# TencentARC/SEED-Story

Hardware: AMD Instinct MI355X
Metric: story-steps/sec (text + 1024x1024 image) (higher is better)
Workload: dtype bf16

## Files before the change

### seed-story_amd/csrc/ss_gemm_common.h

```cpp
#pragma once
#include <type_traits>
#include <utility>

#include "ss_common.h"

namespace ss {

typedef __attribute__((ext_vector_type(4))) uint32_t u32x4_t;
typedef __attribute__((ext_vector_type(8))) uint32_t u32x8_t;
template <int NV> struct Frag { uint4 v[NV]; };
template <typename T> struct OutT { using type = T; };
template <> struct OutT<fp8_t> { using type = bf16_t; };
template <typename T> struct Mma;
template <> struct Mma<bf16_t> {
    static constexpr int kK = 32;
    static constexpr int kEB = 2;
    static constexpr int kNV = 1;
    static __device__ __forceinline__ f32x4_t run(const uint4& a, const uint4& b, f32x4_t c) {
        return __builtin_amdgcn_mfma_f32_16x16x32_bf16(__builtin_bit_cast(bf16x8_t, a),
                                                       __builtin_bit_cast(bf16x8_t, b), c, 0, 0, 0);
    }
    static __device__ __forceinline__ void run_inplace(const uint4& a, const uint4& b, f32x4_t& c) {
        asm volatile("v_mfma_f32_16x16x32_bf16 %0, %1, %2, %0"
                     : "+v"(c)
// ... 49 lines not shown
    const float erf_abs = fmaf(-poly * t, e, 1.0f);
    return 0.5f * v + 0.5f * fabsf(v) * erf_abs;
}
template <typename T> __device__ __forceinline__ float gelu_for(float v) {
    if constexpr (Tr<T>::kVec == 8) return gelu_erf16(v);
    else return gelu_erf(v);
}

constexpr int SS_EPI_INTERNAL_GENERIC = 1 << 30;

struct GemmArgs {
    const void* A = nullptr; const void* W = nullptr; void* C = nullptr; const void* bias = nullptr; const void* residual = nullptr;
    int M = 0, N = 0, K = 0;
    int64_t lda = 0, ldw = 0, ldc = 0, ldr = 0;
    int epi = 0;
    const void* rowvec = nullptr; int rows_per_batch = 1; int64_t rowvec_ld = 0;
    int conv_H = 0, conv_W = 0, conv_Cin = 0, conv_stride = 0, conv_up = 0, conv_Ho = 0, conv_Wo = 0;
    int swz = 0;
    const float* scale_a = nullptr; const float* scale_w = nullptr;
    const float* shift_a = nullptr;
    double* rowstat_out = nullptr;
    float* rowpart = nullptr; int rowpart_ld = 0;
    const float* ln_part = nullptr; int ln_nstrip = 0; float ln_inv_width = 0.f, ln_eps = 0.f;
    int ksplit = 1;
};
static_assert(sizeof(GemmArgs) == 224, "GemmArgs is a kernel argument: its layout does not change");

static inline GemmArgs gemm_args(const void* A, const void* W, void* C, int64_t M, int64_t N, int64_t K, int64_t lda, int64_t ldw,
                          int64_t ldc, int epi, const void* bias = nullptr, const void* residual = nullptr, int64_t ldr = 0) {
    GemmArgs g;
    g.A = A; g.W = W; g.C = C; g.bias = bias; g.residual = residual;
    g.M = (int)M; g.N = (int)N; g.K = (int)K; g.lda = lda; g.ldw = ldw; g.ldc = ldc; g.ldr = ldr; g.epi = epi;
    return g;
}

__device__ __forceinline__ void xcd_tile_id(int swz, int MT, int NT, int id, int& mt, int& nt) {
    if (!swz) { mt = id / NT; nt = id - mt * NT; return; }
    const int total = MT * NT;
    const int xcd = id & 7, j = id >> 3;
    const int base = total >> 3, rem = total & 7;
    const int L = xcd * base + (xcd < rem ? xcd : rem) + j;
    const int GM = swz;
    const int per_group = GM * NT;
    const int gidx = L / per_group, r = L - gidx * per_group;
    const int m0 = gidx * GM;
    const int gm = (MT - m0) < GM ? (MT - m0) : GM;
    nt = r / gm;
    mt = m0 + r - nt * gm;
}
__device__ __forceinline__ void xcd_tile(int swz, int MT, int NT, int& mt, int& nt) {
    xcd_tile_id(swz, MT, NT, blockIdx.y * gridDim.x + blockIdx.x, mt, nt);
}


typedef __attribute__((address_space(3))) void lds_void_t;

__device__ __forceinline__ void dma16(const void* gsrc, uint32_t lds_base) {
    uint32_t keep;
    asm volatile(
        "s_mov_b32 %0, m0\n\t"
        "s_mov_b32 m0, %2\n\t"
        "s_nop 0\n\t"
        "global_load_lds_dwordx4 %1, off\n\t"
        "s_mov_b32 m0, %0"
        : "=&s"(keep)
        : "v"(gsrc), "s"(lds_base)
        : "memory");
}
__device__ __forceinline__ uint32_t m0_save() {
    uint32_t keep;
    asm volatile("s_mov_b32 %0, m0" : "=s"(keep)::"memory");
    return keep;
}
__device__ __forceinline__ void m0_restore(uint32_t keep) { asm volatile("s_mov_b32 m0, %0" ::"s"(keep) : "memory"); }
__device__ __forceinline__ void dma16s(uint32_t voff, const void* sbase, uint32_t lds_base) {
    asm volatile(
        "s_mov_b32 m0, %2\n\t"
        "s_nop 0\n\t"
        "global_load_lds_dwordx4 %0, %1"
        :
        : "v"(voff), "s"(sbase), "s"(lds_base)
        : "memory");
}

__device__ __forceinline__ const char* uniform_ptr(const char* p) {
    const uint64_t v = (uint64_t)(size_t)p;
    const uint32_t lo = __builtin_amdgcn_readfirstlane((uint32_t)v), hi = __builtin_amdgcn_readfirstlane((uint32_t)(v >> 32));
    return (const char*)(size_t)(((uint64_t)hi << 32) | lo);
}

typedef __attribute__((address_space(1))) char gmem_char_t;
typedef __attribute__((address_space(1))) u32x4_t gmem_u32x4_t;
__device__ __forceinline__ uint4 gmem_ld16(const gmem_char_t* p) {
    const u32x4_t v = *reinterpret_cast<const gmem_u32x4_t*>(p);
    return make_uint4(v[0], v[1], v[2], v[3]);
}
__device__ __forceinline__ void gmem_st16(gmem_char_t* p, const uint4& u) {
    const u32x4_t v = {u.x, u.y, u.z, u.w};
    *reinterpret_cast<gmem_u32x4_t*>(p) = v;
}
__device__ __forceinline__ gmem_char_t* uniform_gptr(const char* p) {
    const uint64_t v = (uint64_t)(size_t)p;
    const uint32_t lo = __builtin_amdgcn_readfirstlane((uint32_t)v), hi = __builtin_amdgcn_readfirstlane((uint32_t)(v >> 32));
    return (gmem_char_t*)(size_t)(((uint64_t)hi << 32) | lo);
}

// ... 564 lines not shown
```

### seed-story_amd/csrc/ss_gemm_pp.inc

```

namespace ss {

template <int BN, int FLAGS>
struct PpLds {
    static constexpr int FN = BN / 64, FN0 = (FN + 1) / 2, FN1 = FN / 2, TN = FN * 16;
    static constexpr int HA = 128 * 128, HB0 = 4 * FN0 * 16 * 128, HB1 = 4 * FN1 * 16 * 128;
    static constexpr int BUF = 2 * HA + HB0 + HB1;
    static constexpr int STG_CR = 16, STG_WAVE = STG_CR * (TN * 2 + 16);
    static constexpr bool STG_IN_RING = 2 * BUF + 8 * STG_WAVE > 163840;
    static constexpr int BYTES = 2 * BUF + ((FLAGS & 8) != 0 && !STG_IN_RING ? 8 * STG_WAVE : 0);
};

static __device__ __attribute__((aligned(4096))) unsigned int g_pp_zero_page[1024];

__device__ __forceinline__ void dma16v(const char* gsrc, uint32_t lds_base) {
    asm volatile(
        "s_mov_b32 m0, %1\n\t"
        "s_nop 0\n\t"
        "global_load_lds_dwordx4 %0, off"
        :
        : "v"(gsrc), "s"(lds_base)
        : "memory");
}

template <typename T, int BN, int FLAGS, bool CONV>
__global__ __launch_bounds__(512) void gemm_pp_kernel(const GemmArgs g, const int total_tiles) {
    using Lds = PpLds<BN, FLAGS>;
    constexpr int BM = 256, FN = Lds::FN, FN0 = Lds::FN0, FN1 = Lds::FN1, TM = 128, TN = Lds::TN, FM = 8;
    static_assert(BN == 256 || BN == 320, "tile widths");
    constexpr bool EXACT = BN == 320 || CONV;
    constexpr bool PRIO = (FLAGS & 1) != 0, PERSIST = (FLAGS & 2) != 0, TWO = (FLAGS & 4) != 0, STAGED = (FLAGS & 8) != 0, RSTAT = (FLAGS & 32) != 0;
    constexpr int EM = ((FLAGS & 16) != 0) ? 2 : 0;
    constexpr int HA = Lds::HA, HB0 = Lds::HB0, HB1 = Lds::HB1, BUF = Lds::BUF;
    constexpr int OFF_A0 = 0, OFF_A1 = HA, OFF_B0 = 2 * HA, OFF_B1 = 2 * HA + HB0;
    constexpr int NP0 = FN0, NP1 = FN1;
    constexpr int FLY = NP0 + 2 + NP1;
    constexpr int STG_CR = Lds::STG_CR, STG_WAVE = Lds::STG_WAVE;
    constexpr bool STG_IN_RING = Lds::STG_IN_RING;
    static_assert(!(PERSIST && STG_IN_RING), "persistent tiles prefetch under the epilogue: the strips need their own LDS");
    static_assert(Mma<T>::kEB == 2, "16-bit operands");
    using TO = T;
    extern __shared__ __attribute__((aligned(16))) char smem_raw[];

    const int tid = threadIdx.x, lane = tid & 63;
    const int wid = __builtin_amdgcn_readfirstlane(tid >> 6);
    const int wm = wid >> 2, wn = wid & 3;
    const int l15 = lane & 15, grp = lane >> 4;
    const int M = g.M, N = g.N;
    const int MT = (M + BM - 1) / BM, NT = (N + BN - 1) / BN;
    const int ntiles = g.K / 64;
    const int tpt = CONV ? g.conv_Cin / 64 : 1;
    const uint32_t tpt_inv = CONV ? (65536u + (uint32_t)tpt - 1u) / (uint32_t)tpt : 0u;
    const int lw = CONV ? __builtin_ctz((unsigned)g.conv_W) : 0;
    const uint32_t lds0 = __builtin_amdgcn_readfirstlane((uint32_t)(size_t)(lds_void_t*)smem_raw);

    const int srow = lane >> 3;
    const int schunk = (lane & 7) ^ srow;
    auto b_col = [&](int h, int i) {
        const int RH = (h ? FN1 : FN0) * 16;
        const int r8 = (wid + 8 * i) * 8;
        return (r8 / RH) * TN + (h ? FN0 * 16 : 0) + r8 % RH + srow;
    };
    int m_blk = 0, n_blk = 0;
    uint32_t voffA[EXACT ? 1 : 2][EXACT ? 1 : 2], voffW[EXACT ? 1 : 2][EXACT ? 1 : 3];
    const char* sbaseA = nullptr;
    const char* sbaseW = nullptr;
    auto setup_tile = [&](int vid) {
        int mt_, nt_;
        xcd_tile_id(g.swz, MT, NT, vid, mt_, nt_);
        m_blk = mt_ * BM; n_blk = nt_ * BN;
        if constexpr (CONV) {
            voffA[0][0] = (uint32_t)(srow * g.conv_Cin * 2 + schunk * 16);
            voffW[0][0] = (uint32_t)((int64_t)srow * g.ldw * 2 + schunk * 16);
        } else if constexpr (EXACT) {
            voffA[0][0] = (uint32_t)((int64_t)srow * g.lda * 2 + schunk * 16);
            voffW[0][0] = (uint32_t)((int64_t)srow * g.ldw * 2 + schunk * 16);
        } else {
#pragma unroll
            for (int h = 0; h < 2; ++h) {
#pragma unroll
                for (int i = 0; i < 2; ++i) {
                    int m = m_blk + i * 128 + h * 64 + wid * 8 + srow;
                    m = m < M ? m : M - 1;
                    voffA[h][i] = (uint32_t)((int64_t)(m - m_blk) * g.lda * 2 + schunk * 16);
                }
#pragma unroll
                for (int i = 0; i < (h ? NP1 : NP0); ++i) {
                    int n = n_blk + b_col(h, i);
                    n = n < N ? n : N - 1;
                    voffW[h][i] = (uint32_t)((int64_t)(n - n_blk) * g.ldw * 2 + schunk * 16);
                }
            }
        }
        sbaseA = uniform_ptr((const char*)g.A + (CONV ? (int64_t)0 : (int64_t)m_blk * g.lda * 2));
        sbaseW = uniform_ptr((const char*)g.W + (int64_t)n_blk * g.ldw * 2);
    };
    struct Cur { const char* src; int dy, dx, c, tap; };
    auto cur_set_tap = [&](Cur& k) {
        const int t3 = (k.tap * 11) >> 5;
        k.dy = t3 - 1; k.dx = k.tap - 3 * t3 - 1;
        k.src = (const char*)g.A + ((int64_t)(k.dy * g.conv_W + k.dx) * g.conv_Cin + k.c * 64) * 2;
    };
    auto cur_make = [&](int t) {
        Cur k;
        k.tap = (int)(((uint32_t)t * tpt_inv) >> 16);
        k.c = t - k.tap * tpt;
        cur_set_tap(k);
        return k;
    };
    auto cur_next = [&](Cur& k) {
        k.c += 1; k.src += 128;
        if (k.c == tpt) { k.c = 0; k.tap += 1; cur_set_tap(k); }
    };
    auto stage_conv = [&](const Cur& k, int b, int h) {
        const uint32_t keep = m0_save();
        const uint32_t dst = lds0 + (uint32_t)(b * BUF + (h ? OFF_A1 : OFF_A0) + wid * 1024);
#pragma unroll
        for (int i = 0; i < 2; ++i) {
            const int m0 = m_blk + i * 128 + h * 64 + wid * 8;
            const int y0 = (m0 >> lw) & (g.conv_H - 1), x0 = m0 & (g.conv_W - 1);
            const bool yok = (unsigned)(y0 + k.dy) < (unsigned)g.conv_H;
            const int bad = (k.dx < 0 && x0 == 0) ? 0 : ((k.dx > 0 && x0 + 8 == g.conv_W) ? 7 : -1);
            const char* ps = uniform_ptr(k.src + (int64_t)(m0 * g.conv_Cin * 2));
            const uint32_t d = __builtin_amdgcn_readfirstlane(dst + i * 8192u);
            if (yok && bad < 0) {
                dma16s(voffA[0][0], ps, d);
            } else {
                const bool ok = yok && (lane >> 3) != bad;
                const char* pa = ok ? ps + voffA[0][0] : reinterpret_cast<const char*>(g_pp_zero_page) + ((tid & 255) << 4);
                dma16v(pa, d);
            }
        }
        m0_restore(keep);
    };
    auto stage = [&](int t, int b, int which) {
        const uint32_t keep = m0_save();
        const int h = which & 1;
        if (which < 2) {
            const uint32_t dst = lds0 + (uint32_t)(b * BUF + (h ? OFF_A1 : OFF_A0) + wid * 1024);
            const char* src = sbaseA + (int64_t)t * 128;
#pragma unroll
            for (int i = 0; i < 2; ++i) {
                if constexpr (CONV) {
                } else if constexpr (EXACT)
                    dma16s(voffA[0][0], uniform_ptr(src + (int64_t)(i * 128 + h * 64 + wid * 8) * g.lda * 2), __builtin_amdgcn_readfirstlane(dst + i * 8192u));
                else
                    dma16s(voffA[h][i], src, __builtin_amdgcn_readfirstlane(dst + i * 8192u));
            }
        } else {
            const uint32_t dst = lds0 + (uint32_t)(b * BUF + (h ? OFF_B1 : OFF_B0) + wid * 1024);
            const char* src = sbaseW + (int64_t)t * 128;
#pragma unroll
            for (int i = 0; i < (h ? NP1 : NP0); ++i) {
                if constexpr (EXACT)
                    dma16s(voffW[0][0], uniform_ptr(src + (int64_t)(b_col(h, i) - srow) * g.ldw * 2), __builtin_amdgcn_readfirstlane(dst + i * 8192u));
                else
                    dma16s(voffW[h][i], src, __builtin_amdgcn_readfirstlane(dst + i * 8192u));
            }
        }
        m0_restore(keep);
    };
    auto prologue = [&]() {
        if constexpr (CONV) {
            const Cur k0 = cur_make(0);
            stage(0, 0, 2); stage_conv(k0, 0, 0); stage(0, 0, 3); stage_conv(k0, 0, 1);
            if (ntiles > 1) { stage_conv(cur_make(1), 1, 0); stage(1, 1, 2); if constexpr (!TWO) stage(1, 1, 3); }
        } else {
            stage(0, 0, 2); stage(0, 0, 0); stage(0, 0, 3); stage(0, 0, 1);
            if (ntiles > 1) { stage(1, 1, 0); stage(1, 1, 2); if constexpr (!TWO) stage(1, 1, 3); }
        }
    };

    const uint32_t fsw = (uint32_t)((grp ^ (l15 & 7)) << 4);
    const uint32_t fa0 = (uint32_t)((wm * 64 + l15) * 128) + fsw, fa1 = fa0 ^ 64u;
    const uint32_t fw00 = (uint32_t)((wn * FN0 * 16 + l15) * 128) + fsw, fw01 = fw00 ^ 64u;
    const uint32_t fw10 = (uint32_t)((wn * FN1 * 16 + l15) * 128) + fsw, fw11 = fw10 ^ 64u;
    uint4 fa[4][2], fw0[FN0][2], fw1[FN1][2];
    auto read_a = [&](const char* half) {
#pragma unroll
        for (int j = 0; j < 4; ++j) {
            fa[j][0] = *reinterpret_cast<const uint4*>(half + fa0 + j * 2048);
            fa[j][1] = *reinterpret_cast<const uint4*>(half + fa1 + j * 2048);
        }
    };
    auto read_w0 = [&](const char* half) {
#pragma unroll
        for (int i = 0; i < FN0; ++i) {
            fw0[i][0] = *reinterpret_cast<const uint4*>(half + fw00 + i * 2048);
            fw0[i][1] = *reinterpret_cast<const uint4*>(half + fw01 + i * 2048);
        }
    };
    auto read_w1 = [&](const char* half) {
#pragma unroll
        for (int i = 0; i < FN1; ++i) {
            fw1[i][0] = *reinterpret_cast<const uint4*>(half + fw10 + i * 2048);
            fw1[i][1] = *reinterpret_cast<const uint4*>(half + fw11 + i * 2048);
        }
    };
    f32x4_t acc[FN][FM];
    auto mma = [&](int h, auto hp_tag) {
        constexpr int hp = decltype(hp_tag)::value;
        if constexpr (PRIO) __builtin_amdgcn_s_setprio(1);
#pragma unroll
        for (int ks = 0; ks < 2; ++ks)
#pragma unroll
            for (int i = 0; i < (hp ? FN1 : FN0); ++i)
#pragma unroll
                for (int j = 0; j < 4; ++j) {
                    if constexpr (hp == 0) Mma<T>::run_inplace(fw0[i][ks], fa[j][ks], acc[i][h * 4 + j]);
                    else Mma<T>::run_inplace(fw1[i][ks], fa[j][ks], acc[FN0 + i][h * 4 + j]);
                }
        if constexpr (PRIO) __builtin_amdgcn_s_setprio(0);
    };
    constexpr std::integral_constant<int, 0> H0{};
    constexpr std::integral_constant<int, 1> H1{};
    auto bar = [&]() { __builtin_amdgcn_s_barrier(); };
    auto pin = [&]() { __builtin_amdgcn_sched_barrier(0); };

    int vid = blockIdx.x;
    setup_tile(vid);
    prologue();
    bool first = true;

    while (true) {
        const int m_cur = m_blk, n_cur = n_blk;
        const int vnext = vid + (int)gridDim.x;
        const bool has_next = PERSIST && vnext < total_tiles;
#pragma unroll
        for (int i = 0; i < FN; ++i)
#pragma unroll
            for (int j = 0; j < FM; ++j) acc[i][j] = f32x4_t{0.f, 0.f, 0.f, 0.f};
        if (first && ntiles > 1) wait_vmcnt<(TWO ? 2 + NP0 : FLY)>(); else wait_vmcnt<0>();
        first = false;
        bar();
#pragma unroll
        for (int i = 0; i < FN; ++i)
#pragma unroll
            for (int j = 0; j < FM; ++j) asm volatile("" : "+v"(acc[i][j]));
        asm volatile("s_nop 7" ::: "memory");
        if (wm == 1) bar();
        Cur P1 = cur_make(CONV ? 1 : 0), P2 = cur_make(CONV ? 2 : 0);

        auto tile = [&](int t, auto btag) {
            constexpr int b = decltype(btag)::value;
            const char* L = smem_raw + b * BUF;
            const bool s1 = t + 1 < ntiles, s2 = t + 2 < ntiles;
            read_w0(L + OFF_B0);
            pin();
            read_a(L + OFF_A0);
            pin();
            if (s1) { if constexpr (CONV) stage_conv(P1, b ^ 1, 1); else stage(t + 1, b ^ 1, 1); }
            asm volatile("s_waitcnt lgkmcnt(8)" ::: "memory");
            bar();
            asm volatile("s_waitcnt lgkmcnt(0)" ::: "memory");
            pin();
            mma(0, H0);
            pin();
            bar();
            read_w1(L + OFF_B1);
            pin();
            if (s2) stage(t + 2, b, 2);
            bar();
            asm volatile("s_waitcnt lgkmcnt(0)" ::: "memory");
            pin();
            mma(0, H1);
            pin();
            bar();
            read_a(L + OFF_A1);
            pin();
            if (s2) { if constexpr (CONV) stage_conv(P2, b, 0); else stage(t + 2, b, 0); }
            bar();
            asm volatile("s_waitcnt lgkmcnt(0)" ::: "memory");
            pin();
            mma(1, H1);
            pin();
            bar();
            if (s2) { stage(t + 2, b, 3); wait_vmcnt<FLY>(); } else { wait_vmcnt<0>(); }
            bar();
            pin();
            mma(1, H0);
            pin();
            bar();
            if constexpr (CONV) { P1 = P2; cur_next(P2); }
        };
        auto tile2 = [&](int t, auto btag) {
            constexpr int b = decltype(btag)::value;
            const char* L = smem_raw + b * BUF;
            const bool s1 = t + 1 < ntiles, s2 = t + 2 < ntiles;
            read_w0(L + OFF_B0);
            read_w1(L + OFF_B1);
            read_a(L + OFF_A0);
            pin();
            if (s1) {
                stage(t + 1, b ^ 1, 3);
                if constexpr (CONV) stage_conv(P1, b ^ 1, 1); else stage(t + 1, b ^ 1, 1);
                wait_vmcnt<4 + NP0 + NP1>();
            } else {
                wait_vmcnt<0>();
            }
            asm volatile("s_waitcnt lgkmcnt(0)" ::: "memory");
            bar();
            pin();
            mma(0, H0);
            mma(0, H1);
            pin();
            bar();
            read_a(L + OFF_A1);
            pin();
            if (s2) {
                if constexpr (CONV) stage_conv(P2, b, 0); else stage(t + 2, b, 0);
                stage(t + 2, b, 2);
                wait_vmcnt<4 + NP0>();
            } else if (s1) {
                wait_vmcnt<2>();
            } else {
                wait_vmcnt<0>();
            }
            asm volatile("s_waitcnt lgkmcnt(0)" ::: "memory");
            bar();
            pin();
            mma(1, H1);
            mma(1, H0);
            pin();
            bar();
            if constexpr (CONV) { P1 = P2; cur_next(P2); }
        };
        int t = 0;
        for (; t + 1 < ntiles; t += 2) {
            if constexpr (TWO) { tile2(t, std::integral_constant<int, 0>{}); tile2(t + 1, std::integral_constant<int, 1>{}); }
            else { tile(t, std::integral_constant<int, 0>{}); tile(t + 1, std::integral_constant<int, 1>{}); }
        }
        if (t < ntiles) { if constexpr (TWO) tile2(t, std::integral_constant<int, 0>{}); else tile(t, std::integral_constant<int, 0>{}); }
        if (wm == 0) bar();

        if (has_next) {
            setup_tile(vnext);
            prologue();
        }
        asm volatile("s_nop 15\n\ts_nop 15" ::: "memory");
#pragma unroll
        for (int i = 0; i < FN; ++i)
#pragma unroll
            for (int j = 0; j < FM; ++j) asm volatile("" : "+v"(acc[i][j]));

        bool staged = false;
        if constexpr (STAGED) {
            constexpr size_t A16 = 15;
            staged = (n_cur + wn * TN + TN <= N) && (((size_t)g.C | (size_t)g.residual | (size_t)g.bias | (size_t)g.rowvec) & A16) == 0 &&
                     ((g.ldc | g.ldr | g.rowvec_ld) & 7) == 0 && (EM == 0 || ((size_t)g.scale_w & A16) == 0);
            if (staged) {
                char* strip = smem_raw + (STG_IN_RING ? 0 : 2 * BUF) + wid * STG_WAVE;
                const int mb = m_cur + wm * TM, nb = n_cur + wn * TN;
                const bool o_gelu = (g.epi & SS_EPI_GELU) != 0, o_geglu = (g.epi & SS_EPI_GEGLU_PAIR) != 0;
                const bool o_rv = g.rowvec != nullptr || (!CONV && (g.epi & SS_EPI_INTERNAL_GENERIC) != 0);
                if constexpr (EM == 0 && !RSTAT) {
                    const bool o_res = (g.epi & SS_EPI_RESIDUAL) != 0;
                    if (!o_gelu && !o_geglu && !o_rv && !o_res) gemm_epilogue_staged_pipe<TO, FM, FN, 1, false, EXACT>(g, acc, mb, nb, lane, strip);
                    else if (!o_gelu && !o_geglu && !o_rv) gemm_epilogue_staged_pipe<TO, FM, FN, 1, true, EXACT>(g, acc, mb, nb, lane, strip);
                    else if (CONV && !o_gelu && !o_geglu && !o_res && (g.rows_per_batch & 15) == 0) gemm_epilogue_staged_pipe<TO, FM, FN, 3, false, EXACT>(g, acc, mb, nb, lane, strip);
                    else if (!CONV && o_geglu && !o_gelu && !o_rv && !o_res) gemm_epilogue_staged_pipe<TO, FM, FN, 4, false, EXACT>(g, acc, mb, nb, lane, strip);
                    else if (!CONV && o_gelu && !o_geglu && !o_rv && !o_res) gemm_epilogue_staged_pipe<TO, FM, FN, 2, false, EXACT>(g, acc, mb, nb, lane, strip);
                    else gemm_epilogue_staged<TO, FM, FN, STG_CR, EM, RSTAT, 0>(g, acc, mb, nb, lane, strip);
                } else {
                if (!o_gelu && !o_geglu && !o_rv) gemm_epilogue_staged<TO, FM, FN, STG_CR, EM, RSTAT, 1>(g, acc, mb, nb, lane, strip);
// ... 59 lines not shown
```

### seed-story_amd/csrc/ss_gemm_sp.inc

```

namespace ss {

template <int BM, int BN, int WM, int WN, int NS, int FLAGS>
struct SpLds {
    static constexpr int NW = WM * WN, TILE_BYTES = (BM + BN) * 128;
    static constexpr int STG_CR = 16, STG_WAVE = STG_CR * ((BN / WN) * 2 + 16);
    static constexpr bool STG_IN_RING = (NW == 4 ? 2 : 1) * (NS * TILE_BYTES + NW * STG_WAVE) > 163840;
    static constexpr int BYTES = NS * TILE_BYTES + ((FLAGS & 8) != 0 && !STG_IN_RING ? NW * STG_WAVE : 0);
};

template <typename T, int BM, int BN, int WM, int WN, int NH, int NS, int FLAGS, bool CONV>
__global__ __launch_bounds__(64 * WM * WN) void gemm_sp_kernel(const GemmArgs g, const int total_tiles) {
    constexpr int NW = WM * WN;
    constexpr int TM = BM / WM, TN = BN / WN;
    constexpr int FM = TM / 16, FN = TN / 16;
    constexpr int GA = BM / 8, GW = BN / 8;
    constexpr int IA = (GA + NW - 1) / NW, IW = (GW + NW - 1) / NW;
    constexpr bool EVEN = (GA % NW == 0) && (GW % NW == 0);
    constexpr bool PRIO = (FLAGS & 1) != 0, PERSIST = (FLAGS & 2) != 0, SPREAD = (FLAGS & 4) != 0, STAGED = (FLAGS & 8) != 0;
    constexpr bool RSTAT = (FLAGS & 32) != 0;
    constexpr bool SPLITK = (FLAGS & 64) != 0;
    static_assert(!SPLITK || (!PERSIST && !STAGED && !CONV && !RSTAT && (FLAGS & 16) == 0), "split-K: plain tiles only");
    static_assert(BM % 8 == 0 && BN % 8 == 0 && TM % 16 == 0 && TN % 16 == 0, "tile geometry");
    static_assert(NS == 2 || (NS == 3 && !CONV), "ring depth");
    constexpr int EB = Mma<T>::kEB, KT = 128 / EB, KS = KT / Mma<T>::kK, NV = Mma<T>::kNV;
    constexpr bool F8 = EB == 1;
    static_assert(KS == 2 || (KS == 1 && NS == 2 && !CONV), "fp8 tiles: double-buffered GEMM only");
    static_assert(!F8 || NW % 2 == 0, "fp8 swizzle: DMA groups are dealt to an even number of waves");
    using TO = typename OutT<T>::type;
    constexpr int EM = F8 ? 1 : (((FLAGS & 16) != 0) ? 2 : 0);
    static_assert(!(F8 && (FLAGS & 16)), "fp8 tiles carry their own scaling epilogue");
    extern __shared__ __attribute__((aligned(16))) char smem_raw[];
    using Lds = SpLds<BM, BN, WM, WN, NS, FLAGS>;
    constexpr int TILE_BYTES = Lds::TILE_BYTES, STG_CR = Lds::STG_CR, STG_WAVE = Lds::STG_WAVE;
    constexpr bool STG_IN_RING = Lds::STG_IN_RING;
    constexpr bool PREFETCH_EARLY = !(STAGED && STG_IN_RING);

    const int tid = threadIdx.x, lane = tid & 63;
    const int wid = __builtin_amdgcn_readfirstlane(tid >> 6);
    const int wm = wid / WN, wn = wid % WN;
    const int l15 = lane & 15, grp = lane >> 4;
    const int M = g.M, N = g.N;
    const int MT = (M + BM - 1) / BM, NT = (N + BN - 1) / BN;
    int kt0 = 0, ntiles = g.K / KT;
    if constexpr (SPLITK) {
        const int per = (ntiles + g.ksplit - 1) / g.ksplit;
        kt0 = (int)blockIdx.y * per;
        ntiles = ntiles - kt0 < per ? ntiles - kt0 : per;
        if (ntiles < 0) ntiles = 0;
    }
    const uint32_t lds0 = __builtin_amdgcn_readfirstlane((uint32_t)(size_t)(lds_void_t*)smem_raw);
    const int cntA = EVEN ? IA : (GA - wid + NW - 1) / NW, cntW = EVEN ? IW : (GW - wid + NW - 1) / NW;

    const int srow = lane >> 3;
    const int schunk = F8 ? ((lane & 7) ^ (((srow >> 1) & 1) | ((wid & 1) << 2))) : ((lane & 7) ^ srow);
    int m_blk = 0, n_blk = 0;
    uint32_t voffW[IW], voffA[IA];
    int cbH[IA], cyS[IA], cxS[IA];
    const char* sbaseW = nullptr;
    const char* sbaseA = nullptr;
    auto setup_tile = [&](int vid) {
        int mt_, nt_;
        xcd_tile_id(g.swz, MT, NT, vid, mt_, nt_);
        m_blk = mt_ * BM; n_blk = nt_ * BN;
#pragma unroll
        for (int i = 0; i < IW; ++i) {
            int n = n_blk + (i * NW + wid) * 8 + srow;
            n = n < N ? n : N - 1;
            voffW[i] = (uint32_t)((int64_t)(n - n_blk) * g.ldw * EB + schunk * 16);
        }
        sbaseW = (const char*)g.W + (int64_t)n_blk * g.ldw * EB + (int64_t)kt0 * 128;
        sbaseA = (const char*)g.A + (CONV ? 0 : (int64_t)kt0 * 128);
        if constexpr (CONV) {
            const int hw = g.conv_Ho * g.conv_Wo;
#pragma unroll
            for (int i = 0; i < IA; ++i) {
                int m = m_blk + (i * NW + wid) * 8 + srow;
                m = m < M ? m : M - 1;
                const int b = m / hw;
                const int rem = m - b * hw;
                const int y = rem / g.conv_Wo;
                cbH[i] = b * g.conv_H;
                cyS[i] = y * g.conv_stride;
                cxS[i] = (rem - y * g.conv_Wo) * g.conv_stride;
            }
        } else {
#pragma unroll
            for (int i = 0; i < IA; ++i) {
                int m = m_blk + (i * NW + wid) * 8 + srow;
                m = m < M ? m : M - 1;
                voffA[i] = (uint32_t)((int64_t)(m - m_blk) * g.lda * EB + schunk * 16);
            }
            sbaseA += (int64_t)m_blk * g.lda * EB;
        }
        sbaseW = uniform_ptr(sbaseW);
        sbaseA = uniform_ptr(sbaseA);
    };

    auto issue_piece = [&](int t, int buf, int q) {
        const uint32_t base = lds0 + (uint32_t)(buf * TILE_BYTES);
        if (q < IA) {
            const int i = q;
            if (!(EVEN || i < cntA)) return;
            if constexpr (CONV) {
                const int k0 = t * 64;
                const int tap = k0 / g.conv_Cin;
                const int ci = k0 - tap * g.conv_Cin + schunk * 8;
                const int dy = tap / 3 - 1, dx = tap - (tap / 3) * 3 - 1;
                const int Hin = g.conv_up ? 2 * g.conv_H : g.conv_H, Win = g.conv_up ? 2 * g.conv_W : g.conv_W;
                const int r8 = (i * NW + wid) * 8;
                int iy = cyS[i] + dy, ix = cxS[i] + dx;
                const bool ok = (unsigned)iy < (unsigned)Hin && (unsigned)ix < (unsigned)Win;
                if (g.conv_up) { iy >>= 1; ix >>= 1; }
                const uint32_t off = (uint32_t)((((cbH[i] + iy) * g.conv_W + ix) * g.conv_Cin + ci) * 2);
                if (ok) {
                    dma16s(off, sbaseA, __builtin_amdgcn_readfirstlane(base + (uint32_t)(r8 * 128)));
                } else {
                    *reinterpret_cast<uint4*>(smem_raw + buf * TILE_BYTES + r8 * 128 + lane * 16) = make_uint4(0, 0, 0, 0);
                }
            } else {
                dma16s(voffA[i], sbaseA + (int64_t)t * 128,
                       __builtin_amdgcn_readfirstlane(base + (uint32_t)((i * NW + wid) * 8 * 128)));
            }
        } else {
            const int i = q - IA;
            if (!(EVEN || i < cntW)) return;
            dma16s(voffW[i], sbaseW + (int64_t)t * 128,
                   __builtin_amdgcn_readfirstlane(base + (uint32_t)((BM + (i * NW + wid) * 8) * 128)));
        }
    };
    auto issue_tile = [&](int t, int buf) {
        const uint32_t keep = m0_save();
#pragma unroll
        for (int q = 0; q < IA + IW; ++q) issue_piece(t, buf, q);
        m0_restore(keep);
    };

    auto wait_fly = [&](int fly) {
        if (CONV || fly <= 0) { wait_vmcnt<0>(); return; }
        constexpr int HI = IA + IW;
        const int mine = cntA + cntW;
        if (EVEN || mine == HI) { if (fly == 1) wait_vmcnt<HI>(); else wait_vmcnt<2 * HI>(); }
        else if (mine == HI - 1) { if (fly == 1) wait_vmcnt<HI - 1>(); else wait_vmcnt<2 * (HI - 1)>(); }
        else { if (fly == 1) wait_vmcnt<(HI > 2 ? HI - 2 : 0)>(); else wait_vmcnt<(HI > 2 ? 2 * (HI - 2) : 0)>(); }
    };

    const uint32_t fchunk = F8 ? (uint32_t)(2 * grp) : (uint32_t)grp;
    const uint32_t fswz = F8 ? (uint32_t)(((l15 >> 1) & 1) | (((l15 >> 3) & 1) << 2)) : (uint32_t)(l15 & 7);
    const uint32_t fa0 = (uint32_t)((wm * TM + l15) * 128 + ((fchunk ^ fswz) << 4));
    const uint32_t fw0 = (uint32_t)((BM + wn * TN + l15) * 128 + ((fchunk ^ fswz) << 4));
    constexpr int FMH = FM / NH, P = KS * NH;
    static_assert(FM % NH == 0, "A fragments must split evenly");
    Frag<NV> fa[2][FMH], fw[2][FN];
    auto read_phase = [&](int buf, int p, int par) {
        const int ks = p / NH, h = p % NH;
        const int sa = (par * P + p) & 1, sw = (par * KS + ks) & 1;
        const char* b = smem_raw + buf * TILE_BYTES;
        const uint32_t xa = ks ? (fa0 ^ 64u) : fa0, xw = ks ? (fw0 ^ 64u) : fw0;
        if (h == 0) {
#pragma unroll
            for (int i = 0; i < FN; ++i) {
                fw[sw][i].v[0] = *reinterpret_cast<const uint4*>(b + xw + i * 2048);
                if constexpr (NV == 2) fw[sw][i].v[1] = *reinterpret_cast<const uint4*>(b + (xw ^ 16u) + i * 2048);
            }
        }
#pragma unroll
        for (int j = 0; j < FMH; ++j) {
            fa[sa][j].v[0] = *reinterpret_cast<const uint4*>(b + xa + (h * FMH + j) * 2048);
            if constexpr (NV == 2) fa[sa][j].v[1] = *reinterpret_cast<const uint4*>(b + (xa ^ 16u) + (h * FMH + j) * 2048);
        }
    };

    f32x4_t acc[FN][FM];
    const uint32_t mma_aux = Mma<T>::make_aux();
    auto mma_phase = [&](int p, int par) {
        const int ks = p / NH, h = p % NH;
        const int sa = (par * P + p) & 1, sw = (par * KS + ks) & 1;
#pragma unroll
        for (int i = 0; i < FN; ++i)
#pragma unroll
// ... 99 lines not shown
#pragma unroll
        for (int i = 0; i < FN; ++i)
#pragma unroll
            for (int j = 0; j < FM; ++j) asm volatile("" : "+v"(acc[i][j]));

        bool staged = false;
        if constexpr (STAGED) {
            constexpr size_t A16 = 15;
            staged = (n_cur + wn * TN + TN <= N) && (((size_t)g.C | (size_t)g.residual | (size_t)g.bias | (size_t)g.rowvec) & A16) == 0 &&
                     ((g.ldc | g.ldr | g.rowvec_ld) & 7) == 0 && (EM == 0 || ((size_t)g.scale_w & A16) == 0);
            if constexpr (STG_IN_RING) {
                asm volatile("s_waitcnt lgkmcnt(0)" ::: "memory");
                __syncthreads();
            }
            if (staged) {
                char* strip = smem_raw + (STG_IN_RING ? 0 : NS * TILE_BYTES) + wid * STG_WAVE;
                const int mb = m_cur + wm * TM, nb = n_cur + wn * TN;
                const bool o_gelu = (g.epi & SS_EPI_GELU) != 0, o_geglu = (g.epi & SS_EPI_GEGLU_PAIR) != 0;
                const bool o_rv = g.rowvec != nullptr || (!CONV && (g.epi & SS_EPI_INTERNAL_GENERIC) != 0);
                if (!o_gelu && !o_geglu && !o_rv) {
                    gemm_epilogue_staged<TO, FM, FN, STG_CR, EM, RSTAT, 1>(g, acc, mb, nb, lane, strip);
                } else if constexpr (CONV) {
                    gemm_epilogue_staged<TO, FM, FN, STG_CR, EM, RSTAT, 3>(g, acc, mb, nb, lane, strip);
                } else {
                    if (o_geglu && !o_gelu && !o_rv) gemm_epilogue_staged<TO, FM, FN, STG_CR, EM, RSTAT, 4>(g, acc, mb, nb, lane, strip);
                    else if (o_gelu && !o_geglu && !o_rv) gemm_epilogue_staged<TO, FM, FN, STG_CR, EM, RSTAT, 2>(g, acc, mb, nb, lane, strip);
                    else gemm_epilogue_staged<TO, FM, FN, STG_CR, EM, RSTAT, 0>(g, acc, mb, nb, lane, strip);
                }
            }
        }
        if constexpr (SPLITK) gemm_epilogue_partial<FM, FN>(g, acc, m_cur + wm * TM, n_cur + wn * TN, l15, grp, (int)blockIdx.y);
        else if (!staged) gemm_epilogue<TO, FM, FN, EM, RSTAT>(g, acc, m_cur + wm * TM, n_cur + wn * TN, l15, grp);
        if (!has_next) break;
        if constexpr (!PREFETCH_EARLY) {
            asm volatile("s_waitcnt lgkmcnt(0)" ::: "memory");
            __syncthreads();
            setup_tile(vnext);
#pragma unroll
            for (int st = 0; st < NS; ++st)
                if (st < ntiles) issue_tile(st, st);
        }
        vid = vnext;
    }
}

template <typename T, int BM, int BN, int WM, int WN, int NH, int NS_, int FLAGS>
static int sp_launch(const GemmArgs& g, hipStream_t s) {
    constexpr bool CONV = SS_SP_CONV != 0;
    constexpr int NS = CONV ? 2 : NS_;
    const bool conv = g.conv_Cin > 0;
    if (conv != CONV) return 1;
    constexpr int KT = 128 / Mma<T>::kEB;
    const bool ok = (g.K % KT == 0) && (!conv || g.conv_Cin % 64 == 0) && g.K >= KT &&
                    (conv ? (int64_t)g.M * g.conv_stride * g.conv_stride * g.conv_Cin * 2 < (1ll << 31)
                          : ((int64_t)BM * g.lda * Mma<T>::kEB < (1ll << 31))) && (int64_t)BN * g.ldw * Mma<T>::kEB < (1ll << 31);
    if (!ok) return 1;
    if ((g.rowstat_out || g.rowpart) && !(FLAGS & 32)) return 1;
    constexpr size_t lds = SpLds<BM, BN, WM, WN, NS, FLAGS>::BYTES;
    if ((g.ksplit > 1) != ((FLAGS & 64) != 0)) return 1;
    const int cap = (FLAGS & 2) ? num_cus() * (lds > 80 * 1024 ? 1 : 2) : 0;
    return launch_tiles<gemm_sp_kernel<T, BM, BN, WM, WN, NH, NS, FLAGS, CONV>>("gemm_sp", g, cdiv(g.M, BM) * cdiv(g.N, BN), cap,
                                                                                64 * WM * WN, lds, s);
}

#define SS_SP_CASE(id, BM, BN, WM, WN, NH, NS, FLAGS, VAR) case id: return sp_launch<T, BM, BN, WM, WN, NH, NS, FLAGS>(g, s);
#define SS_SP_VARIANT(HAS, ID, BM, BN, WM, WN, NH, NS, FLAGS) \
    if constexpr ((HAS) != 0) { if (cfg == (ID)) return sp_launch<T, BM, BN, WM, WN, NH, NS, FLAGS>(g, s); }
#define SS_SP_LNFOLD(id, BM, BN, WM, WN, NH, NS, FLAGS, VAR) SS_SP_VARIANT((VAR) & 1, (id) + 100, BM, BN, WM, WN, NH, NS, (FLAGS) | 16)
#define SS_SP_ROWSTAT(id, BM, BN, WM, WN, NH, NS, FLAGS, VAR) SS_SP_VARIANT((VAR) & 2, (id) + 200, BM, BN, WM, WN, NH, NS, (FLAGS) | 32)
#if defined(SS_SP_FP8)
int gemm_sp_dispatch_fp8(int cfg, const GemmArgs& g, hipStream_t s) {
    using T = fp8_t;
    switch (cfg) {
        SS_SP_FP8_TILES(SS_SP_CASE)
        default: return 1;
    }
}
#else
#if SS_SP_CONV
template <typename T> int gemm_sp_dispatch_conv(int cfg, const GemmArgs& g, hipStream_t s) {
#else
template <typename T> int gemm_sp_dispatch(int cfg, const GemmArgs& g, hipStream_t s) {
#endif
    switch (cfg) {
        SS_SP_TILES(SS_SP_CASE)
#if !SS_SP_CONV
        SS_SP_SPLITK_TILES(SS_SP_CASE)
#endif
        default: break;
    }
#if !SS_SP_CONV
    SS_SP_TILES(SS_SP_ROWSTAT)
    SS_SP_TILES(SS_SP_LNFOLD)
#endif
    return 1;
}

#if SS_SP_CONV
template int gemm_sp_dispatch_conv<SS_SP_T>(int, const GemmArgs&, hipStream_t);
#else
template int gemm_sp_dispatch<SS_SP_T>(int, const GemmArgs&, hipStream_t);
#endif
#endif

}
```

### seed-story_amd/csrc/ss_gemm_w4.inc

```

namespace ss {

typedef __attribute__((ext_vector_type(16))) float f32x16_t;

template <int... Is, typename F>
__device__ __forceinline__ void w4_static_for_impl(std::integer_sequence<int, Is...>, F&& f) {
    (f(std::integral_constant<int, Is>{}), ...);
}
template <int N, typename F>
__device__ __forceinline__ void w4_static_for(F&& f) {
    w4_static_for_impl(std::make_integer_sequence<int, N>{}, static_cast<F&&>(f));
}

template <int NV> struct W4Frag { uint4 v[NV]; };
template <typename T> struct Mma32;
template <> struct Mma32<bf16_t> {
    static constexpr int kEB = 2, kKS = 4, kNV = 1;
    static __device__ __forceinline__ uint32_t make_aux() { return 0u; }
    static __device__ __forceinline__ void run(const W4Frag<1>& w, const W4Frag<1>& a, f32x16_t& c, uint32_t) {
        asm volatile("v_mfma_f32_32x32x16_bf16 %0, %1, %2, %0"
                     : "+a"(c)
                     : "v"(__builtin_bit_cast(u32x4_t, w.v[0])), "v"(__builtin_bit_cast(u32x4_t, a.v[0])));
    }
};
// ... 157 lines not shown
    const uint32_t lds0 = __builtin_amdgcn_readfirstlane((uint32_t)(size_t)(lds_void_t*)smem_raw);

    const int srow = lane >> 3;
    const int schunk = (lane & 7) ^ ((4 * (wid & 1) + (srow >> 1)) & 7);
    int m_blk = 0, n_blk = 0;
    uint32_t voffW[IW], voffA[IA];
    int cbH[CONV ? IA : 1], cyS[CONV ? IA : 1], cxS[CONV ? IA : 1];
    const char* sbaseW = nullptr;
    const char* sbaseA = nullptr;
    auto setup_tile = [&](int vid) {
        int mt_, nt_;
        xcd_tile_id(g.swz, MT, NT, vid, mt_, nt_);
        m_blk = mt_ * BM; n_blk = nt_ * BN;
#pragma unroll
        for (int i = 0; i < IW; ++i) {
            int n = n_blk + (i * 4 + wid) * 8 + srow;
            n = n < N ? n : N - 1;
            voffW[i] = (uint32_t)((int64_t)(n - n_blk) * g.ldw * EB + schunk * 16);
        }
        sbaseW = (const char*)g.W + (int64_t)n_blk * g.ldw * EB;
        sbaseA = (const char*)g.A;
        if constexpr (CONV) {
            const int hw = g.conv_Ho * g.conv_Wo;
#pragma unroll
            for (int i = 0; i < IA; ++i) {
                int m = m_blk + (i * 4 + wid) * 8 + srow;
                m = m < M ? m : M - 1;
                const int b = m / hw;
                const int rem = m - b * hw;
                const int y = rem / g.conv_Wo;
                cbH[i] = b * g.conv_H;
                cyS[i] = y * g.conv_stride;
                cxS[i] = (rem - y * g.conv_Wo) * g.conv_stride;
            }
        } else {
#pragma unroll
            for (int i = 0; i < IA; ++i) {
                int m = m_blk + (i * 4 + wid) * 8 + srow;
                m = m < M ? m : M - 1;
                voffA[i] = (uint32_t)((int64_t)(m - m_blk) * g.lda * EB + schunk * 16);
            }
            sbaseA += (int64_t)m_blk * g.lda * EB;
        }
        sbaseW = uniform_ptr(sbaseW);
        sbaseA = uniform_ptr(sbaseA);
    };

    auto issue_piece = [&](int t, int slot, int q) {
        const uint32_t base = lds0 + (uint32_t)slot * (uint32_t)TILE_BYTES;
        if (q < IA) {
            const int i = q;
            const int r8 = (i * 4 + wid) * 8;
            if constexpr (CONV) {
                const int k0 = t * 64;
                const int tap = k0 / g.conv_Cin;
                const int ci = k0 - tap * g.conv_Cin + schunk * 8;
                const int dy = tap / 3 - 1, dx = tap - (tap / 3) * 3 - 1;
                const int Hin = g.conv_up ? 2 * g.conv_H : g.conv_H, Win = g.conv_up ? 2 * g.conv_W : g.conv_W;
                int iy = cyS[i] + dy, ix = cxS[i] + dx;
                const bool ok = (unsigned)iy < (unsigned)Hin && (unsigned)ix < (unsigned)Win;
                if (g.conv_up) { iy >>= 1; ix >>= 1; }
                const uint32_t off = (uint32_t)((((cbH[i] + iy) * g.conv_W + ix) * g.conv_Cin + ci) * 2);
                if (ok) {
                    dma16s(off, sbaseA, __builtin_amdgcn_readfirstlane(base + (uint32_t)(r8 * 128)));
                } else {
                    *reinterpret_cast<uint4*>(smem_raw + slot * TILE_BYTES + r8 * 128 + lane * 16) = make_uint4(0, 0, 0, 0);
                }
            } else {
                dma16s(voffA[i], sbaseA + (int64_t)t * 128, __builtin_amdgcn_readfirstlane(base + (uint32_t)(r8 * 128)));
            }
        } else {
            const int i = q - IA;
            dma16s(voffW[i], sbaseW + (int64_t)t * 128,
                   __builtin_amdgcn_readfirstlane(base + (uint32_t)((BM + (i * 4 + wid) * 8) * 128)));
        }
    };
    auto issue_range = [&](int t, int slot, int q0, int q1) {
        const uint32_t keep = m0_save();
#pragma unroll
        for (int q = 0; q < NP; ++q)
            if (q >= q0 && q < q1) issue_piece(t, slot, q);
        m0_restore(keep);
    };

    const uint32_t fsw = (uint32_t)(((lane & 31) >> 1) & 7);
    const uint32_t fc0 = ((uint32_t)((lane >> 5) << (F8 ? 1 : 0)) ^ fsw) << 4;
    const uint32_t fa0 = (uint32_t)((wm * TM + (lane & 31)) * 128) + fc0;
    const uint32_t fw0 = (uint32_t)((BM + wn * TN + (lane & 31)) * 128) + fc0;
    W4Frag<NV> fa[2][NBM], fw[2][NBN];
    auto read_one = [&](int slot, int ks, int set, int r) {
        const char* b = smem_raw + slot * TILE_BYTES;
        const uint32_t x = (uint32_t)ks << (F8 ? 6 : 5);
        auto rd = [&](W4Frag<NV>& f, uint32_t addr) {
            f.v[0] = *reinterpret_cast<const uint4*>(b + addr);
            if constexpr (NV == 2) f.v[1] = *reinterpret_cast<const uint4*>(b + (addr ^ 16u));
        };
        if (r == 0) rd(fw[set][0], fw0 ^ x);
        else if (r <= NBM) rd(fa[set][r - 1], (fa0 ^ x) + (r - 1) * 4096);
        else rd(fw[set][r - NBM], (fw0 ^ x) + (r - NBM) * 4096);
    };

    f32x16_t acc[NBN][NBM];
    const uint32_t mma_aux = Mma32<T>::make_aux();

    auto kstep = [&](auto set_tag, auto early_tag, int rslot, int rks, auto nd_tag, auto d0_tag, bool dma_on, int dt, int dslot) {
        constexpr int set = decltype(set_tag)::value;
        constexpr bool EARLY = decltype(early_tag)::value;
        constexpr int ND = decltype(nd_tag)::value, DQ0 = decltype(d0_tag)::value;
        const uint32_t keep = m0_save();
        w4_static_for<NQ>([&](auto q_tag) {
            constexpr int q = decltype(q_tag)::value;
            constexpr int bn = q / NBM, bm = q % NBM;
            Mma32<T>::run(fw[set][bn], fa[set][bm], acc[bn][bm], mma_aux);
#pragma unroll
            for (int r = 0; r < NR; ++r) {
                const int gq = EARLY ? r : (r * NQ) / NR;
                if (gq == q) read_one(rslot, rks, set ^ 1, r);
            }
#pragma unroll
            for (int d = 0; d < ND; ++d) {
                const int gq = ((2 * d + 1) * NQ) / (2 * ND > 0 ? 2 * ND : 1);
                if (gq == q) { if (dma_on) issue_piece(dt, dslot, DQ0 + d); }
            }
            __builtin_amdgcn_sched_barrier(0);
        });
        m0_restore(keep);
// ... 146 lines not shown
```

Before: 2.344.

## Reorder conv implicit-GEMM K loop to iterate taps inside channel chunks

Result: no change. 2.353, median of 6 (+0.4%).

```diff
diff --git a/seed-story_amd/csrc/ss_gemm_common.h b/seed-story_amd/csrc/ss_gemm_common.h
--- a/seed-story_amd/csrc/ss_gemm_common.h
+++ b/seed-story_amd/csrc/ss_gemm_common.h
@@ -125,6 +125,29 @@
     xcd_tile_id(swz, MT, NT, blockIdx.y * gridDim.x + blockIdx.x, mt, nt);
 }
 
+
+struct ConvKTile {
+    int tap, dy, dx;
+    int c;
+    int a_off;
+    int w_off;
+};
+__device__ __forceinline__ ConvKTile conv_ktile_at(int c, int tap, int Cin, int Win) {
+    ConvKTile k;
+    const int t3 = (tap * 11) >> 5;
+    k.tap = tap; k.c = c;
+    k.dy = t3 - 1; k.dx = tap - 3 * t3 - 1;
+    k.a_off = ((k.dy * Win + k.dx) * Cin + c * 64) * 2;
+    k.w_off = (tap * Cin + c * 64) * 2;
+    return k;
+}
+__device__ __forceinline__ ConvKTile conv_ktile(int t, int Cin, int Win) {
+    const int c = (int)((unsigned)t / 9u);
+    return conv_ktile_at(c, t - 9 * c, Cin, Win);
+}
+__device__ __forceinline__ ConvKTile conv_ktile_next(const ConvKTile& k, int Cin, int Win) {
+    return k.tap == 8 ? conv_ktile_at(k.c + 1, 0, Cin, Win) : conv_ktile_at(k.c, k.tap + 1, Cin, Win);
+}
 
 typedef __attribute__((address_space(3))) void lds_void_t;
 
diff --git a/seed-story_amd/csrc/ss_gemm_pp.inc b/seed-story_amd/csrc/ss_gemm_pp.inc
--- a/seed-story_amd/csrc/ss_gemm_pp.inc
+++ b/seed-story_amd/csrc/ss_gemm_pp.inc
@@ -49,8 +49,6 @@
     const int M = g.M, N = g.N;
     const int MT = (M + BM - 1) / BM, NT = (N + BN - 1) / BN;
     const int ntiles = g.K / 64;
-    const int tpt = CONV ? g.conv_Cin / 64 : 1;
-    const uint32_t tpt_inv = CONV ? (65536u + (uint32_t)tpt - 1u) / (uint32_t)tpt : 0u;
     const int lw = CONV ? __builtin_ctz((unsigned)g.conv_W) : 0;
     const uint32_t lds0 = __builtin_amdgcn_readfirstlane((uint32_t)(size_t)(lds_void_t*)smem_raw);
 
@@ -95,23 +93,9 @@
         sbaseA = uniform_ptr((const char*)g.A + (CONV ? (int64_t)0 : (int64_t)m_blk * g.lda * 2));
         sbaseW = uniform_ptr((const char*)g.W + (int64_t)n_blk * g.ldw * 2);
     };
-    struct Cur { const char* src; int dy, dx, c, tap; };
-    auto cur_set_tap = [&](Cur& k) {
-        const int t3 = (k.tap * 11) >> 5;
-        k.dy = t3 - 1; k.dx = k.tap - 3 * t3 - 1;
-        k.src = (const char*)g.A + ((int64_t)(k.dy * g.conv_W + k.dx) * g.conv_Cin + k.c * 64) * 2;
-    };
-    auto cur_make = [&](int t) {
-        Cur k;
-        k.tap = (int)(((uint32_t)t * tpt_inv) >> 16);
-        k.c = t - k.tap * tpt;
-        cur_set_tap(k);
-        return k;
-    };
-    auto cur_next = [&](Cur& k) {
-        k.c += 1; k.src += 128;
-        if (k.c == tpt) { k.c = 0; k.tap += 1; cur_set_tap(k); }
-    };
+    using Cur = ConvKTile;
+    auto cur_make = [&](int t) { return conv_ktile(t, g.conv_Cin, g.conv_W); };
+    auto cur_next = [&](Cur& k) { k = conv_ktile_next(k, g.conv_Cin, g.conv_W); };
     auto stage_conv = [&](const Cur& k, int b, int h) {
         const uint32_t keep = m0_save();
         const uint32_t dst = lds0 + (uint32_t)(b * BUF + (h ? OFF_A1 : OFF_A0) + wid * 1024);
@@ -121,7 +105,7 @@
             const int y0 = (m0 >> lw) & (g.conv_H - 1), x0 = m0 & (g.conv_W - 1);
             const bool yok = (unsigned)(y0 + k.dy) < (unsigned)g.conv_H;
             const int bad = (k.dx < 0 && x0 == 0) ? 0 : ((k.dx > 0 && x0 + 8 == g.conv_W) ? 7 : -1);
-            const char* ps = uniform_ptr(k.src + (int64_t)(m0 * g.conv_Cin * 2));
+            const char* ps = uniform_ptr((const char*)g.A + k.a_off + (int64_t)(m0 * g.conv_Cin * 2));
             const uint32_t d = __builtin_amdgcn_readfirstlane(dst + i * 8192u);
             if (yok && bad < 0) {
                 dma16s(voffA[0][0], ps, d);
@@ -133,12 +117,12 @@
         }
         m0_restore(keep);
     };
-    auto stage = [&](int t, int b, int which) {
+    auto stage_at = [&](int64_t koff, int b, int which) {
         const uint32_t keep = m0_save();
         const int h = which & 1;
         if (which < 2) {
             const uint32_t dst = lds0 + (uint32_t)(b * BUF + (h ? OFF_A1 : OFF_A0) + wid * 1024);
-            const char* src = sbaseA + (int64_t)t * 128;
+            const char* src = sbaseA + koff;
 #pragma unroll
             for (int i = 0; i < 2; ++i) {
                 if constexpr (CONV) {
@@ -149,7 +133,7 @@
             }
         } else {
             const uint32_t dst = lds0 + (uint32_t)(b * BUF + (h ? OFF_B1 : OFF_B0) + wid * 1024);
-            const char* src = sbaseW + (int64_t)t * 128;
+            const char* src = sbaseW + koff;
 #pragma unroll
             for (int i = 0; i < (h ? NP1 : NP0); ++i) {
                 if constexpr (EXACT)
@@ -160,11 +144,13 @@
         }
         m0_restore(keep);
     };
+    auto stage = [&](int t, int b, int which) { stage_at((int64_t)t * 128, b, which); };
+    auto stage_w = [&](const Cur& k, int b, int h) { stage_at((int64_t)k.w_off, b, 2 + h); };
     auto prologue = [&]() {
         if constexpr (CONV) {
-            const Cur k0 = cur_make(0);
-            stage(0, 0, 2); stage_conv(k0, 0, 0); stage(0, 0, 3); stage_conv(k0, 0, 1);
-            if (ntiles > 1) { stage_conv(cur_make(1), 1, 0); stage(1, 1, 2); if constexpr (!TWO) stage(1, 1, 3); }
+            const Cur k0 = cur_make(0), k1 = cur_make(1);
+            stage_w(k0, 0, 0); stage_conv(k0, 0, 0); stage_w(k0, 0, 1); stage_conv(k0, 0, 1);
+            if (ntiles > 1) { stage_conv(k1, 1, 0); stage_w(k1, 1, 0); if constexpr (!TWO) stage_w(k1, 1, 1); }
         } else {
             stage(0, 0, 2); stage(0, 0, 0); stage(0, 0, 3); stage(0, 0, 1);
             if (ntiles > 1) { stage(1, 1, 0); stage(1, 1, 2); if constexpr (!TWO) stage(1, 1, 3); }
@@ -259,7 +245,7 @@
             bar();
             read_w1(L + OFF_B1);
             pin();
-            if (s2) stage(t + 2, b, 2);
+            if (s2) { if constexpr (CONV) stage_w(P2, b, 0); else stage(t + 2, b, 2); }
             bar();
             asm volatile("s_waitcnt lgkmcnt(0)" ::: "memory");
             pin();
@@ -275,7 +261,7 @@
             mma(1, H1);
             pin();
             bar();
-            if (s2) { stage(t + 2, b, 3); wait_vmcnt<FLY>(); } else { wait_vmcnt<0>(); }
+            if (s2) { if constexpr (CONV) stage_w(P2, b, 1); else stage(t + 2, b, 3); wait_vmcnt<FLY>(); } else { wait_vmcnt<0>(); }
             bar();
             pin();
             mma(1, H0);
@@ -292,8 +278,8 @@
             read_a(L + OFF_A0);
             pin();
             if (s1) {
-                stage(t + 1, b ^ 1, 3);
-                if constexpr (CONV) stage_conv(P1, b ^ 1, 1); else stage(t + 1, b ^ 1, 1);
+                if constexpr (CONV) { stage_w(P1, b ^ 1, 1); stage_conv(P1, b ^ 1, 1); }
+                else { stage(t + 1, b ^ 1, 3); stage(t + 1, b ^ 1, 1); }
                 wait_vmcnt<4 + NP0 + NP1>();
             } else {
                 wait_vmcnt<0>();
@@ -308,8 +294,8 @@
             read_a(L + OFF_A1);
             pin();
             if (s2) {
-                if constexpr (CONV) stage_conv(P2, b, 0); else stage(t + 2, b, 0);
-                stage(t + 2, b, 2);
+                if constexpr (CONV) { stage_conv(P2, b, 0); stage_w(P2, b, 0); }
+                else { stage(t + 2, b, 0); stage(t + 2, b, 2); }
                 wait_vmcnt<4 + NP0>();
             } else if (s1) {
                 wait_vmcnt<2>();
diff --git a/seed-story_amd/csrc/ss_gemm_sp.inc b/seed-story_amd/csrc/ss_gemm_sp.inc
--- a/seed-story_amd/csrc/ss_gemm_sp.inc
+++ b/seed-story_amd/csrc/ss_gemm_sp.inc
@@ -56,7 +56,7 @@
     const int schunk = F8 ? ((lane & 7) ^ (((srow >> 1) & 1) | ((wid & 1) << 2))) : ((lane & 7) ^ srow);
     int m_blk = 0, n_blk = 0;
     uint32_t voffW[IW], voffA[IA];
-    int cbH[IA], cyS[IA], cxS[IA];
+    int cbH[IA], cyxS[IA];
     const char* sbaseW = nullptr;
     const char* sbaseA = nullptr;
     auto setup_tile = [&](int vid) {
@@ -81,8 +81,7 @@
                 const int rem = m - b * hw;
                 const int y = rem / g.conv_Wo;
                 cbH[i] = b * g.conv_H;
-                cyS[i] = y * g.conv_stride;
-                cxS[i] = (rem - y * g.conv_Wo) * g.conv_stride;
+                cyxS[i] = ((y * g.conv_stride) << 16) | ((rem - y * g.conv_Wo) * g.conv_stride);
             }
         } else {
 #pragma unroll
@@ -99,17 +98,21 @@
 
     auto issue_piece = [&](int t, int buf, int q) {
         const uint32_t base = lds0 + (uint32_t)(buf * TILE_BYTES);
+        int kc = 0, kdy = 0, kdx = 0, kw = 0;
+        if constexpr (CONV) {
+            const ConvKTile kt = conv_ktile(kt0 + t, g.conv_Cin, g.conv_W);
+            kc = __builtin_amdgcn_readfirstlane(kt.c * 64); kdy = __builtin_amdgcn_readfirstlane(kt.dy);
+            kdx = __builtin_amdgcn_readfirstlane(kt.dx); kw = __builtin_amdgcn_readfirstlane(kt.w_off);
+        }
         if (q < IA) {
             const int i = q;
             if (!(EVEN || i < cntA)) return;
             if constexpr (CONV) {
-                const int k0 = t * 64;
-                const int tap = k0 / g.conv_Cin;
-                const int ci = k0 - tap * g.conv_Cin + schunk * 8;
-                const int dy = tap / 3 - 1, dx = tap - (tap / 3) * 3 - 1;
+                const int ci = kc + schunk * 8;
+                const int dy = kdy, dx = kdx;
                 const int Hin = g.conv_up ? 2 * g.conv_H : g.conv_H, Win = g.conv_up ? 2 * g.conv_W : g.conv_W;
                 const int r8 = (i * NW + wid) * 8;
-                int iy = cyS[i] + dy, ix = cxS[i] + dx;
+                int iy = (cyxS[i] >> 16) + dy, ix = (cyxS[i] & 0xffff) + dx;
                 const bool ok = (unsigned)iy < (unsigned)Hin && (unsigned)ix < (unsigned)Win;
                 if (g.conv_up) { iy >>= 1; ix >>= 1; }
                 const uint32_t off = (uint32_t)((((cbH[i] + iy) * g.conv_W + ix) * g.conv_Cin + ci) * 2);
@@ -125,7 +128,8 @@
         } else {
             const int i = q - IA;
             if (!(EVEN || i < cntW)) return;
-            dma16s(voffW[i], sbaseW + (int64_t)t * 128,
+            const int64_t koff = CONV ? (int64_t)kw : (int64_t)t * 128;
+            dma16s(voffW[i], sbaseW + koff,
                    __builtin_amdgcn_readfirstlane(base + (uint32_t)((BM + (i * NW + wid) * 8) * 128)));
         }
     };
@@ -331,7 +335,8 @@
     if (conv != CONV) return 1;
     constexpr int KT = 128 / Mma<T>::kEB;
     const bool ok = (g.K % KT == 0) && (!conv || g.conv_Cin % 64 == 0) && g.K >= KT &&
-                    (conv ? (int64_t)g.M * g.conv_stride * g.conv_stride * g.conv_Cin * 2 < (1ll << 31)
+                    (conv ? (int64_t)g.M * g.conv_stride * g.conv_stride * g.conv_Cin * 2 < (1ll << 31) &&
+                                (g.conv_H << g.conv_up) < 32768 && (g.conv_W << g.conv_up) < 32768
                           : ((int64_t)BM * g.lda * Mma<T>::kEB < (1ll << 31))) && (int64_t)BN * g.ldw * Mma<T>::kEB < (1ll << 31);
     if (!ok) return 1;
     if ((g.rowstat_out || g.rowpart) && !(FLAGS & 32)) return 1;
diff --git a/seed-story_amd/csrc/ss_gemm_w4.inc b/seed-story_amd/csrc/ss_gemm_w4.inc
--- a/seed-story_amd/csrc/ss_gemm_w4.inc
+++ b/seed-story_amd/csrc/ss_gemm_w4.inc
@@ -233,10 +233,9 @@
             const int i = q;
             const int r8 = (i * 4 + wid) * 8;
             if constexpr (CONV) {
-                const int k0 = t * 64;
-                const int tap = k0 / g.conv_Cin;
-                const int ci = k0 - tap * g.conv_Cin + schunk * 8;
-                const int dy = tap / 3 - 1, dx = tap - (tap / 3) * 3 - 1;
+                const ConvKTile kt = conv_ktile(t, g.conv_Cin, g.conv_W);
+                const int ci = kt.c * 64 + schunk * 8;
+                const int dy = kt.dy, dx = kt.dx;
                 const int Hin = g.conv_up ? 2 * g.conv_H : g.conv_H, Win = g.conv_up ? 2 * g.conv_W : g.conv_W;
                 int iy = cyS[i] + dy, ix = cxS[i] + dx;
                 const bool ok = (unsigned)iy < (unsigned)Hin && (unsigned)ix < (unsigned)Win;
@@ -252,7 +251,8 @@
             }
         } else {
             const int i = q - IA;
-            dma16s(voffW[i], sbaseW + (int64_t)t * 128,
+            const int64_t koff = CONV ? (int64_t)conv_ktile(t, g.conv_Cin, g.conv_W).w_off : (int64_t)t * 128;
+            dma16s(voffW[i], CONV ? uniform_ptr(sbaseW + koff) : sbaseW + koff,
                    __builtin_amdgcn_readfirstlane(base + (uint32_t)((BM + (i * 4 + wid) * 8) * 128)));
         }
     };
```
